# burn-research/OpenMEASURE

Measured on AMD Instinct MI355X. Metric: SPR fit+reconstruct throughput (GB/s snapshot matrix), higher is better.
Workload: dtype f64

## Files before the change

### include/spr_hip.h

```cpp
#ifndef SPR_HIP_H
#define SPR_HIP_H

#include <stddef.h>
#include <stdint.h>

#ifdef __cplusplus
extern "C" {
#endif

#define SPR_OK 0
#define SPR_E_INVALID (-1)
#define SPR_E_UNSUPPORTED (-2)
#define SPR_E_HIP (-3)
#define SPR_E_WORKSPACE (-4)

#define SPR_MAX_M 256
#define SPR_MAX_M_WIDE 512
#define SPR_MAX_R 128
#define SPR_MAX_R_STREAM 256
#define SPR_MAX_R_WIDE 1024

#define SPR_ABI_VERSION 5
int spr_abi_version(void);
const char *spr_last_error(void);
int spr_device_cus(int *out_cus);
int spr_upload_bytes(void *d_dst, const void *h_pinned_src, int64_t n_bytes, void *stream);
int spr_download_bytes(void *h_pinned_dst, const void *d_src, int64_t n_bytes, void *h_pinned_ticket, uint64_t ticket_value,
                       void *stream);
int spr_host_tridiag_vectors(const double *h_d, const double *h_e, int32_t m, const double *h_lam, int32_t r, double *h_Z,
                             int32_t iterations);
int spr_host_eig_top(const double *h_G, int32_t m, int32_t r, double *h_lam, double *h_V, void *fn_dsytrd, void *fn_dsterf,
                     void *fn_dormtr);
int spr_host_svd_top(const double *h_M, int32_t m, int32_t r, double *h_S, double *h_V, void *fn_dgebrd, void *fn_dbdsdc,
                     void *fn_dormbr);

size_t spr_stats_gram_workspace(int32_t m, int32_t n_features);
int spr_stats_gram_f64(const double *d_X, int64_t n_rows, int32_t m, int64_t ldx,
                       int64_t row0, int64_t n_points, int32_t n_features, int32_t center,
                       double *d_rowmean, void *d_workspace, size_t workspace_bytes, void *stream);
int spr_stats_gram_finalize_f64(int64_t n_rows, int32_t m, int64_t row0, int64_t n_points,
                                int32_t n_features, const void *d_workspace, size_t workspace_bytes,
                                double *d_fstats, double *d_gram, int32_t ldg, int32_t origin,
                                void *stream);
size_t spr_rowstats_workspace(int32_t n_features);
int spr_rowstats_f64(const double *d_X, int64_t n_rows, int32_t m, int64_t ldx, int64_t row0,
                     int64_t n_points, int32_t n_features, double *d_rowmean, double *d_fstats,
                     void *d_workspace, size_t workspace_bytes, void *stream);
size_t spr_gram_cross_workspace(int32_t m, int32_t n_features);
int spr_gram_cross_f64(const double *d_X, int64_t n_rows, int32_t m, int64_t ldx, int64_t row0,
                       int64_t n_points, int32_t n_features, int32_t center, double *d_rowmean,
                       double *d_gram, void *d_workspace, size_t workspace_bytes, void *stream);
int spr_rowmean_stats_f64(const double *d_rowmean, int64_t n_rows, int64_t row0, int64_t n_points,
                          int32_t n_features, double *d_fstats, void *d_workspace, size_t workspace_bytes,
                          void *stream);
int spr_gram_cross_pair_f64(const double *d_X, int64_t n_rows, int32_t col_a, int32_t col_b, int32_t w_b,
                            int32_t ldg, int64_t ldx, int64_t row0, int64_t n_points, int32_t n_features,
                            int32_t center, double *d_rowmean, double *d_gram, void *d_workspace,
                            size_t workspace_bytes, void *stream);

int32_t spr_spectrum_max_m(void);
int spr_spectrum_f64(const double *d_gram, const double *d_fstats_all, int32_t n_ranks,
                     int32_t n_features, int32_t m, int32_t scale_code, int32_t r, double *d_feat,
                     double *d_scale, double *d_inv_scale, double *d_lam, double *d_S, double *d_expvar,
                     double *d_V, double *d_W, double *d_Ar, double *d_info, void *stream);

int spr_gram_combine_f64(const double *d_gram, const double *d_fstats_all, int32_t n_ranks,
                         int32_t n_features, int32_t m, int32_t scale_code, double *d_G, double *d_feat,
                         double *d_scale, double *d_inv_scale, void *stream);

int spr_stats_gram_shifted_f64(const double *d_X, int64_t n_rows, int32_t m, int64_t ldx, int64_t row0,
                               int64_t n_points, int32_t n_features, const double *d_shift, double *d_rowsum,
                               void *d_workspace, size_t workspace_bytes, void *stream);
int spr_gram_shift_finish_f64(double *d_rowmean, const double *d_rowsum_b, int64_t n_rows, int32_t w_a, int32_t m,
                              double *d_gram, int32_t n_features, void *stream);

int spr_project_f64(const double *d_X, int64_t n_rows, int32_t m, int64_t ldx,
// ... 275 lines not shown
```

### openmeasure_amd/_lib.py

```python
from __future__ import annotations

import ctypes as C
import os

_HERE = os.path.dirname(os.path.abspath(__file__))
LIB_PATH = os.environ.get('SPR_HIP_LIBRARY') or os.path.join(_HERE, 'libspr_hip.so')

SPR_ABI_VERSION = 5
SPR_MAX_M = 256
SPR_MAX_M_WIDE = 512
SPR_MAX_R = 128
SPR_MAX_R_STREAM = 256
SPR_MAX_R_WIDE = 1024

_i32, _i64, _u64, _sz = C.c_int32, C.c_int64, C.c_uint64, C.c_size_t
_p = C.c_void_p
_dbl = C.c_double

PROTOTYPES = {
    'spr_abi_version': (C.c_int, []),
    'spr_last_error': (C.c_char_p, []),
    'spr_device_cus': (C.c_int, [C.POINTER(C.c_int)]),
    'spr_upload_bytes': (C.c_int, [_p, _p, _i64, _p]),
    'spr_download_bytes': (C.c_int, [_p, _p, _i64, _p, _u64, _p]),
    'spr_host_tridiag_vectors': (C.c_int, [_p, _p, _i32, _p, _i32, _p, _i32]),
    'spr_host_eig_top': (C.c_int, [_p, _i32, _i32, _p, _p, _p, _p, _p]),
    'spr_host_svd_top': (C.c_int, [_p, _i32, _i32, _p, _p, _p, _p, _p]),
    'spr_stats_gram_workspace': (_sz, [_i32, _i32]),
    'spr_stats_gram_f64': (C.c_int, [_p, _i64, _i32, _i64, _i64, _i64, _i32, _i32, _p, _p, _sz, _p]),
    'spr_stats_gram_finalize_f64': (C.c_int, [_i64, _i32, _i64, _i64, _i32, _p, _sz, _p, _p, _i32, _i32, _p]),
    'spr_stats_gram_shifted_f64': (C.c_int, [_p, _i64, _i32, _i64, _i64, _i64, _i32, _p, _p, _p, _sz, _p]),
    'spr_gram_shift_finish_f64': (C.c_int, [_p, _p, _i64, _i32, _i32, _p, _i32, _p]),
    'spr_rowstats_workspace': (_sz, [_i32]),
    'spr_rowstats_f64': (C.c_int, [_p, _i64, _i32, _i64, _i64, _i64, _i32, _p, _p, _p, _sz, _p]),
    'spr_gram_cross_workspace': (_sz, [_i32, _i32]),
    'spr_gram_cross_f64': (C.c_int, [_p, _i64, _i32, _i64, _i64, _i64, _i32, _i32, _p, _p, _p, _sz, _p]),
    'spr_gram_cross_pair_f64': (C.c_int, [_p, _i64, _i32, _i32, _i32, _i32, _i64, _i64, _i64, _i32, _i32, _p, _p, _p, _sz, _p]),
    'spr_rowmean_stats_f64': (C.c_int, [_p, _i64, _i64, _i64, _i32, _p, _p, _sz, _p]),
    'spr_spectrum_max_m': (_i32, []),
    'spr_spectrum_f64': (C.c_int, [_p, _p, _i32, _i32, _i32, _i32, _i32, _p, _p, _p, _p, _p, _p, _p, _p, _p, _p, _p]),
    'spr_gram_combine_f64': (C.c_int, [_p, _p, _i32, _i32, _i32, _i32, _p, _p, _p, _p, _p]),
    'spr_project_f64': (C.c_int, [_p, _i64, _i32, _i64, _i64, _i64, _i32, _i32, _p, _p, _p, _i32, _p, _i64, _i32, _p]),
    'spr_project_norms_supported': (_i32, [_i32, _i32, _i64, _i64, _p, _i32]),
    'spr_project_norms_f64': (C.c_int, [_p, _i64, _i32, _i64, _i64, _i64, _i32, _i32, _p, _p, _p, _i32, _p, _i64, _p, _p]),
    'spr_project_stream_norms_f64': (C.c_int, [_p, _i64, _i32, _i64, _i64, _i64, _i32, _i32, _p, _p, _p, _i32, _p, _i64, _p, _p, _sz, _p]),
    'spr_project_stream_workspace': (_sz, [_i32, _i32, _i32]),
    'spr_project_stream_f64': (C.c_int, [_p, _i64, _i32, _i64, _i64, _i64, _i32, _i32, _p, _p, _p, _i32, _p, _i64, _p, _sz, _p]),
    'spr_scale_rows_f64': (C.c_int, [_p, _i64, _i32, _i64, _i64, _i64, _i32, _p, _p, _p, _i64, _p]),
    'spr_unscale_f64': (C.c_int, [_p, _i64, _i64, _i64, _i32, _p, _p, _p, _p, _p]),
    'spr_feature_minmax_workspace': (_sz, [_i32]),
    'spr_feature_minmax_f64': (C.c_int, [_p, _i64, _i32, _i64, _i64, _i64, _i32, _p, _p, _sz, _p]),
    'spr_feature_digit_hist_f64': (C.c_int, [_p, _i64, _i32, _i64, _i64, _i64, _i32, _p, _i32, _i32, _i32, _p, _p]),
    'spr_colsums_workspace': (_sz, [_i32, _i32]),
    'spr_colsums_f64': (C.c_int, [_p, _i64, _i32, _i64, _i64, _i64, _i32, _p, _p, _p, _sz, _p]),
    'spr_fill_feature_f64': (C.c_int, [_p, _i64, _i64, _i64, _i32, _p, _p]),
    'spr_reconstruct_f64': (C.c_int, [_p, _i64, _i32, _i64, _i64, _i64, _i32, _p, _p, _p, _p, _i32, _p, _i64, _p]),
    'spr_bound_sweep_workspace': (_sz, [_i32, _i32]),
    'spr_bound_sweep_f64': (C.c_int, [_p, _i64, _i32, _i64, _i64, _i64, _i32, _p, _p, _p, _p, _p, _i32, _dbl, _i32, _p, _p, _sz, _p]),
    'spr_field_unstage_f64': (C.c_int, [_p, _i32, _i32, _i64, _p, _i64, _p]),
    'spr_field_unstage_blocks_f64': (C.c_int, [_p, _i32, _i32, _i64, _p, _p, _i64, _p]),
    'spr_p2p_handle_bytes': (_sz, []),
    'spr_p2p_alloc': (C.c_int, [_sz, _i32, _p, _p]),
    'spr_p2p_free': (C.c_int, [_p]),
# ... 109 lines not shown
```

### openmeasure_amd/csrc/common.hpp

```cpp
#pragma once
#include <hip/hip_runtime.h>
#include <stdint.h>
#include <stdio.h>

#include "spr_hip.h"

typedef double f64x4 __attribute__((ext_vector_type(4)));
typedef double f64x2 __attribute__((ext_vector_type(2)));

void spr_set_error(const char *fmt, ...);

#define SPR_REQUIRE(cond, code, ...)      \
  do {                                    \
    if (!(cond)) {                        \
      spr_set_error(__VA_ARGS__);         \
      return (code);                      \
    }                                     \
  } while (0)

#define SPR_HIP_TRY(expr)                                                          \
  do {                                                                             \
    hipError_t e__ = (expr);                                                       \
    if (e__ != hipSuccess) {                                                       \
      spr_set_error("%s failed: %s (%s:%d)", #expr, hipGetErrorString(e__),       \
// ... 42 lines not shown
__host__ __device__ inline int seg_first_feature(const SegPlan &p) { return (int)(p.row0 / p.n_points); }
__host__ __device__ inline int seg_last_feature(const SegPlan &p) {
  int64_t f = (p.row0 + p.n_rows - 1) / p.n_points;
  if (f > p.n_features - 1) f = p.n_features - 1;
  return (int)f;
}

inline int seg_total_wgs(const SegPlan &p) {
  int tot = 0;
  for (int f = seg_first_feature(p); f <= seg_last_feature(p); ++f) {
    int64_t lo, hi;
    seg_range(p, f, lo, hi);
    tot += seg_wgs(p, hi - lo);
  }
  return tot;
}

__device__ inline bool seg_locate(const SegPlan &p, int b, int &f, int &wl, int &wpf, int &base,
                                  int64_t &lo, int64_t &hi) {
  int acc = 0;
  int f1 = seg_last_feature(p);
  for (int ff = seg_first_feature(p); ff <= f1; ++ff) {
    seg_range(p, ff, lo, hi);
    int w = seg_wgs(p, hi - lo);
    if (b < acc + w) {
      f = ff; wl = b - acc; wpf = w; base = acc;
      return true;
    }
    acc += w;
  }
  return false;
}

template <int CTRL>
__device__ inline double dpp_f64(double v) {
  union { double d; int i[2]; } a, b;
  a.d = v;
  b.i[0] = __builtin_amdgcn_update_dpp(0, a.i[0], CTRL, 0xF, 0xF, true);
  b.i[1] = __builtin_amdgcn_update_dpp(0, a.i[1], CTRL, 0xF, 0xF, true);
  return b.d;
}

template <int WIDTH>
__device__ inline double group_sum_t(double v) {
  if (WIDTH >= 2) v += dpp_f64<0xB1>(v);
  if (WIDTH >= 4) v += dpp_f64<0x4E>(v);
  if (WIDTH >= 8) v += dpp_f64<0x141>(v);
  if (WIDTH >= 16) v += dpp_f64<0x140>(v);
  if (WIDTH >= 32) v += __shfl_xor(v, 16, 64);
  if (WIDTH >= 64) v += __shfl_xor(v, 32, 64);
  return v;
}

__device__ inline double group_sum(double v, int width) {
  for (int o = width >> 1; o > 0; o >>= 1) v += __shfl_xor(v, o, 64);
  return v;
}

constexpr int spr_pow2_divisor_le64(int n) {
  int p = 1;
  while (p < 64 && n % (2 * p) == 0) p *= 2;
  return p;
}

inline int spr_round_mt(int m) {
  static const int sup[] = {1, 2, 3, 4, 6, 8, 12, 16};
// ... 6 lines not shown
```

### openmeasure_amd/csrc/runtime.hip

```cpp
#include <stdarg.h>
#include <stdlib.h>
#include <string.h>

#include "common.hpp"

namespace {
thread_local char g_err[512] = "";
}

void spr_set_error(const char *fmt, ...) {
  va_list ap;
  va_start(ap, fmt);
  vsnprintf(g_err, sizeof(g_err), fmt, ap);
  va_end(ap);
}

int spr_cached_cus() {
  static int cus = 0;
  if (cus) return cus;
  int dev = 0;
  hipDeviceProp_t prop;
  if (hipGetDevice(&dev) != hipSuccess || hipGetDeviceProperties(&prop, dev) != hipSuccess) return 0;
  cus = prop.multiProcessorCount;
  if (const char *e = getenv("SPR_RESERVE_CUS")) {
    const int k = atoi(e);
    if (k > 0 && k < cus) cus -= k;
  }
  return cus;
}

extern "C" int spr_abi_version(void) { return SPR_ABI_VERSION; }

extern "C" const char *spr_last_error(void) { return g_err; }

extern "C" int spr_device_cus(int *out_cus) {
  SPR_REQUIRE(out_cus != nullptr, SPR_E_INVALID, "spr_device_cus: NULL output");
  const int c = spr_cached_cus();
  SPR_REQUIRE(c > 0, SPR_E_HIP, "spr_device_cus: no HIP device");
  *out_cus = c;
  return SPR_OK;
}

namespace {
__global__ __launch_bounds__(256) void upload_kernel(const uint64_t *__restrict__ src, uint64_t *__restrict__ dst,
                                                     int64_t n_words) {
  for (int64_t i = (int64_t)blockIdx.x * 256 + threadIdx.x; i < n_words; i += (int64_t)gridDim.x * 256)
    dst[i] = __builtin_nontemporal_load(src + i);
}
}

extern "C" int spr_upload_bytes(void *d_dst, const void *h_pinned_src, int64_t n_bytes, void *stream) {
  SPR_REQUIRE(d_dst && h_pinned_src, SPR_E_INVALID, "spr_upload_bytes: NULL pointer");
  SPR_REQUIRE(n_bytes > 0 && n_bytes % 8 == 0, SPR_E_INVALID, "spr_upload_bytes: n_bytes=%lld must be a positive multiple of 8",
              (long long)n_bytes);
  SPR_REQUIRE(((uintptr_t)d_dst | (uintptr_t)h_pinned_src) % 8 == 0, SPR_E_INVALID, "spr_upload_bytes: unaligned pointer");
  const int64_t words = n_bytes / 8;
  int64_t blocks = (words + 255) / 256;
  if (blocks > 64) blocks = 64;
  hipLaunchKernelGGL(upload_kernel, dim3((unsigned)blocks), dim3(256), 0, static_cast<hipStream_t>(stream),
                     static_cast<const uint64_t *>(h_pinned_src), static_cast<uint64_t *>(d_dst), words);
  SPR_LAUNCH_CHECK();
  return SPR_OK;
}

namespace {
__global__ __launch_bounds__(1024) void download_kernel(const uint64_t *__restrict__ src, uint64_t *__restrict__ dst,
                                                        int64_t n_words, unsigned long long *__restrict__ ticket,
                                                        unsigned long long value) {
  for (int64_t i = threadIdx.x; i < n_words; i += 1024) __builtin_nontemporal_store(src[i], dst + i);
  __builtin_amdgcn_fence(__ATOMIC_RELEASE, "");
  __syncthreads();
  if (threadIdx.x == 0) __hip_atomic_store(ticket, value, __ATOMIC_RELEASE, __HIP_MEMORY_SCOPE_SYSTEM);
}
// ... 16 lines not shown
```

### openmeasure_amd/csrc/stats_gram.hip

```cpp
#include <stdlib.h>

#include <type_traits>

#include "rowtile.hpp"

#ifndef GRAM_UNIT_PAIRING
#define GRAM_UNIT_PAIRING 1
#endif
#ifndef GRAM_ABLATE
#define GRAM_ABLATE 0
#endif
#if GRAM_ABLATE == 1
#define GRAM_MFMA(a, b, c) ({ asm volatile("" ::"v"(a), "v"(b)); (c); })
#else
#define GRAM_MFMA(a, b, c) __builtin_amdgcn_mfma_f64_16x16x4f64((a), (b), (c), 0, 0, 0)
#endif

namespace {

template <int MT>
struct GramShape {
  static constexpr int MPAD = 16 * MT;
  static constexpr int MP = MPAD + ((MT % 2 == 0) ? 16 : 0);
  static constexpr int T = MT * (MT + 1) / 2;
  static constexpr int NU = (MT + 1) / 2;
};

template <int MT> struct GramCfg;
template <> struct GramCfg<1>  { static constexpr int NW = 8,  R = 64, KS = 8; static constexpr bool DBUF = true; static constexpr int LPRMAX = 16; };
template <> struct GramCfg<2>  { static constexpr int NW = 8,  R = 32, KS = 8; static constexpr bool DBUF = true; static constexpr int LPRMAX = 16; };
template <> struct GramCfg<3>  { static constexpr int NW = 8,  R = 64, KS = 4; static constexpr bool DBUF = true; static constexpr int LPRMAX = 16; };
#ifndef GRAM4_R
#define GRAM4_R 64
#define GRAM4_LPR 8
#endif
template <> struct GramCfg<4>  { static constexpr int NW = 8,  R = GRAM4_R, KS = 4; static constexpr bool DBUF = true; static constexpr int LPRMAX = GRAM4_LPR; };
template <> struct GramCfg<6>  { static constexpr int NW = 12, R = 48, KS = 4; static constexpr bool DBUF = true; static constexpr int LPRMAX = 16; };
template <> struct GramCfg<8>  { static constexpr int NW = 8,  R = 32, KS = 2; static constexpr bool DBUF = true; static constexpr int LPRMAX = 16; };
template <> struct GramCfg<12> { static constexpr int NW = 12, R = 24, KS = 2; static constexpr bool DBUF = false; static constexpr int LPRMAX = 32; };
#ifndef GRAM_DBUF16
#define GRAM_DBUF16 false
#endif
template <> struct GramCfg<16> { static constexpr int NW = 8,  R = 32, KS = 1; static constexpr bool DBUF = GRAM_DBUF16; static constexpr int LPRMAX = 16; };

template <int MT> struct GramOut { static constexpr int KSO = (GramCfg<MT>::KS >= 4) ? 1 : GramCfg<MT>::KS; };

constexpr int tri_index(int mt, int ti, int tj) { return ti * mt - ti * (ti - 1) / 2 + (tj - ti); }

template <int MT>
__device__ inline void tile_coords(int idx, int &ti, int &tj) {
  ti = 0;
  while (ti < MT - 1 && idx >= MT - ti) { idx -= MT - ti; ++ti; }
  tj = ti + idx;
  if (tj > MT - 1) tj = MT - 1;
}

template <int MT, int U, int VEC, typename TX>
__device__ inline void gram_wave(const TX *__restrict__ X, int64_t ldx, int m, int center,
                                 int64_t lo, int64_t hi, int wl, int wpf, int ks, int wave, int lane,
                                 double *__restrict__ lds0, double *__restrict__ lds1,
                                 double *__restrict__ rowmean, double *__restrict__ stat_part,
                                 double *__restrict__ slab, double *__restrict__ rowsum) {
  using S = GramShape<MT>;
  using C = GramCfg<MT>;
  constexpr int R = C::R, KS = C::KS, NW = C::NW, MP = S::MP, T = S::T;
  constexpr int KROWS = R / KS, KSTEPS = KROWS / 4;
  constexpr int RA = U, RB = MT - 1 - U;
  constexpr int NA = MT - RA;
  constexpr int NB = (RB != RA) ? MT - RB : 0;
  static_assert(KROWS % 4 == 0, "k slice must be a multiple of the MFMA depth");
  using RT = RowTile<MT, R, MP, NW, C::LPRMAX, TX>;

  f64x4 accA[NA];
  f64x4 accB[NB > 0 ? NB : 1];
#pragma unroll
  for (int j = 0; j < NA; ++j) accA[j] = (f64x4){0.0, 0.0, 0.0, 0.0};
#pragma unroll
  for (int j = 0; j < NB; ++j) accB[j] = (f64x4){0.0, 0.0, 0.0, 0.0};

  RowStats st;
  st.init();
  RT tile;

  const int64_t nchunks = (hi - lo + R - 1) / R;
  int64_t c = wl;
  const double *mean_in = rowmean;
  tile.template load<VEC>(X, ldx, m, lo + c * R, hi, wave, lane, mean_in);
  tile.template center_store<true>(lds0, m, center, lo + c * R, hi, wave, lane, rowmean, &st, rowsum);
  int64_t cn = c + wpf;
  int64_t nrow0 = (cn < nchunks) ? lo + cn * R : hi;
  tile.template load<VEC>(X, ldx, m, nrow0, hi, wave, lane, mean_in);
  int buf = 0;
  const int frag = (lane >> 4) * MP + (lane & 15) + ks * KROWS * MP + RA * 16;
  while (c < nchunks) {
    double *cur = buf ? lds1 : lds0;
// ... 57 lines not shown
  if constexpr (KSO != KS) {
    static_assert((size_t)T * 256 <= (size_t)2 * R * MP, "tile staging must fit the panel buffers");
    double *red = lds0 + lane;
    for (int s = KS - 1; s >= 1; --s) {
      __syncthreads();
      if (ks == s) {
#pragma unroll
        for (int j = 0; j < NA; ++j) {
          double *tp = red + tri_index(MT, RA, RA + j) * 256;
          tp[0] = accA[j].x; tp[64] = accA[j].y; tp[128] = accA[j].z; tp[192] = accA[j].w;
        }
#pragma unroll
        for (int j = 0; j < NB; ++j) {
          double *tp = red + tri_index(MT, RB, RB + j) * 256;
          tp[0] = accB[j].x; tp[64] = accB[j].y; tp[128] = accB[j].z; tp[192] = accB[j].w;
        }
      }
      __syncthreads();
      if (ks == s - 1) {
#pragma unroll
        for (int j = 0; j < NA; ++j) {
          const double *tp = red + tri_index(MT, RA, RA + j) * 256;
          accA[j].x += tp[0]; accA[j].y += tp[64]; accA[j].z += tp[128]; accA[j].w += tp[192];
        }
#pragma unroll
        for (int j = 0; j < NB; ++j) {
          const double *tp = red + tri_index(MT, RB, RB + j) * 256;
          accB[j].x += tp[0]; accB[j].y += tp[64]; accB[j].z += tp[128]; accB[j].w += tp[192];
        }
      }
    }
  }
  if (KSO == KS || ks == 0) {
    double *sp = slab + ((int64_t)blockIdx.x * KSO + (KSO == KS ? ks : 0)) * T * 256 + lane;
#pragma unroll
    for (int j = 0; j < NA; ++j) {
      double *tp = sp + (int64_t)tri_index(MT, RA, RA + j) * 256;
      tp[0] = accA[j].x; tp[64] = accA[j].y; tp[128] = accA[j].z; tp[192] = accA[j].w;
    }
#pragma unroll
    for (int j = 0; j < NB; ++j) {
      double *tp = sp + (int64_t)tri_index(MT, RB, RB + j) * 256;
      tp[0] = accB[j].x; tp[64] = accB[j].y; tp[128] = accB[j].z; tp[192] = accB[j].w;
    }
  }
  if ((lane % RT::LPR) == 0) {
    double *q = stat_part + ((int64_t)blockIdx.x * RT::ROWS_PER_IT + wave * RT::RPW + lane / RT::LPR) * 3;
    q[0] = st.cnt; q[1] = st.mean(); q[2] = st.m2();
  }
}

__device__ inline void chan_merge(double &n, double &mu, double &m2, double nb, double mb, double sb) {
  if (nb > 0.0) {
    const double tot = n + nb, d = mb - mu;
    mu += d * nb / tot;
    m2 += sb + d * d * n * nb / tot;
    n = tot;
  }
}

template <int MT, int U, typename TX, bool EXT, bool SUMS>
__device__ inline void gram_wave_own(const TX *__restrict__ X, int64_t ldx, int64_t lo, int64_t hi, int wl, int wpf, int ks,
                                     int wave, int lane, double *__restrict__ lds0, double *__restrict__ lds1,
                                     double *__restrict__ rowmean, double *__restrict__ slab, double *__restrict__ rowsum) {
  using S = GramShape<MT>;
  using C = GramCfg<MT>;
  constexpr int R = C::R, KS = C::KS, NW = C::NW, MP = S::MP, T = S::T;
  constexpr int KROWS = R / KS, KSTEPS = KROWS / 4;
  constexpr int RA = U, RB = MT - 1 - U;
  constexpr int NA = MT - RA;
  constexpr int NB = (RB != RA) ? MT - RB : 0;
  using RT = RowTile<MT, R, MP, NW, C::LPRMAX, TX>;

  f64x4 accA[NA];
  f64x4 accB[NB > 0 ? NB : 1];
#pragma unroll
  for (int j = 0; j < NA; ++j) accA[j] = (f64x4){0.0, 0.0, 0.0, 0.0};
#pragma unroll
  for (int j = 0; j < NB; ++j) accB[j] = (f64x4){0.0, 0.0, 0.0, 0.0};

  RT tile;
  const int64_t nchunks = (hi - lo + R - 1) / R;
  const int64_t lane_off = (int64_t)(wave * RT::RPW + lane / RT::LPR) * ldx;
  auto base_of = [&](int64_t row0) { return X + row0 * ldx; };
  int64_t c = wl;
  int64_t crow0 = lo + c * R;
#pragma unroll
  for (int it = 0; it < RT::IT; ++it) tile.template load_pass_own<EXT>(it, base_of(crow0), ldx, lane_off, hi - crow0, wave, lane, rowmean, crow0);
  if (crow0 + R <= hi) {
#pragma unroll
    for (int it = 0; it < RT::IT; ++it) tile.template center_store_own<true, EXT, SUMS>(it, lds0, crow0, hi - crow0, wave, lane, rowmean, rowsum);
  } else {
#pragma unroll
    for (int it = 0; it < RT::IT; ++it) tile.template center_store_own<false, EXT, SUMS>(it, lds0, crow0, hi - crow0, wave, lane, rowmean, rowsum);
  }
  int64_t cn = c + wpf;
  int64_t nrow0 = (cn < nchunks) ? lo + cn * R : hi;
// ... 23 lines not shown
      double op[2][NA];
#pragma unroll
      for (int j = 0; j < NA; ++j) op[0][j] = p[16 * j];
#pragma unroll
      for (int k = 0; k < KSTEPS; ++k) {
        if (k + 1 < KSTEPS) {
#pragma unroll
          for (int j = 0; j < NA; ++j) op[(k + 1) & 1][j] = p[(k + 1) * 4 * MP + 16 * j];
        }
#pragma unroll
        for (int j = 0; j < NA; ++j) accA[j] = GRAM_MFMA(op[k & 1][0], op[k & 1][j], accA[j]);
#pragma unroll
        for (int j = 0; j < NB; ++j) accB[j] = GRAM_MFMA(op[k & 1][RB - RA], op[k & 1][RB - RA + j], accB[j]);
        if (nfull) stage(std::true_type{}, k); else stage(std::false_type{}, k);
      }
    } else {
#pragma unroll
      for (int k = 0; k < KSTEPS; ++k) {
        double op[NA];
#pragma unroll
        for (int j = 0; j < NA; ++j) op[j] = p[k * 4 * MP + 16 * j];
#pragma unroll
        for (int j = 0; j < NA; ++j) accA[j] = GRAM_MFMA(op[0], op[j], accA[j]);
#pragma unroll
        for (int j = 0; j < NB; ++j) accB[j] = GRAM_MFMA(op[RB - RA], op[RB - RA + j], accB[j]);
        if (nfull) stage(std::true_type{}, k); else stage(std::false_type{}, k);
      }
    }
    buf ^= 1;
    c = cn;
    cn = c2;
    nrow0 = n2row0;
  }
  double *sp = slab + ((int64_t)blockIdx.x * KS + ks) * T * 256 + lane;
#pragma unroll
  for (int j = 0; j < NA; ++j) {
    double *tp = sp + (int64_t)tri_index(MT, RA, RA + j) * 256;
    tp[0] = accA[j].x; tp[64] = accA[j].y; tp[128] = accA[j].z; tp[192] = accA[j].w;
  }
#pragma unroll
  for (int j = 0; j < NB; ++j) {
    double *tp = sp + (int64_t)tri_index(MT, RB, RB + j) * 256;
    tp[0] = accB[j].x; tp[64] = accB[j].y; tp[128] = accB[j].z; tp[192] = accB[j].w;
  }
}

template <int MT, typename TX, bool EXT, bool SUMS>
__global__ __launch_bounds__(GramCfg<MT>::NW * 64) void stats_gram_own_kernel(
    const TX *__restrict__ X, int64_t ldx, SegPlan plan, double *__restrict__ rowmean, double *__restrict__ slab,
    double *__restrict__ rowsum) {
  using S = GramShape<MT>;
  using C = GramCfg<MT>;
  constexpr int NU = S::NU;
  __shared__ double lds[2][C::R * S::MP];
  int f, wl, wpf, base;
  int64_t lo, hi;
  if (!seg_locate(plan, blockIdx.x, f, wl, wpf, base, lo, hi)) return;
  const int lane = threadIdx.x & 63;
  const int wave = __builtin_amdgcn_readfirstlane(threadIdx.x >> 6);
  const int ks = wave / NU;
  const int unit = (GRAM_UNIT_PAIRING && NU == 8 && C::KS == 1) ? ((wave < 4) ? wave : 11 - wave) : wave % NU;
#define GRAM_UNIT(UV)                                                                                          \
  case UV:                                                                                                     \
    if constexpr (UV < NU)                                                                                     \
      gram_wave_own<MT, UV, TX, EXT, SUMS>(X, ldx, lo, hi, wl, wpf, ks, wave, lane, lds[0], lds[1], rowmean, slab, rowsum); \
    break;
  switch (unit) {
    GRAM_UNIT(0) GRAM_UNIT(1) GRAM_UNIT(2) GRAM_UNIT(3) GRAM_UNIT(4) GRAM_UNIT(5) GRAM_UNIT(6) GRAM_UNIT(7)
    default: break;
  }
#undef GRAM_UNIT
}

constexpr int RS_THREADS = 1024;
__global__ __launch_bounds__(RS_THREADS) void gram_rowmean_stats_kernel(const double *__restrict__ rowmean, SegPlan plan,
                                                                        int slots_per_wg, double *__restrict__ stat_part) {
  __shared__ double sn[RS_THREADS / 64], smu[RS_THREADS / 64], sm2[RS_THREADS / 64];
  int f, wl, wpf, base;
  int64_t lo, hi;
  if (!seg_locate(plan, blockIdx.x, f, wl, wpf, base, lo, hi)) return;
  const int lane = threadIdx.x & 63, wave = threadIdx.x >> 6;
  RowStats st;
  st.init();
  const int64_t step = (int64_t)wpf * RS_THREADS;
  int64_t row = lo + (int64_t)wl * RS_THREADS + threadIdx.x;
  for (; row + 3 * step < hi; row += 4 * step) {
    const double a = rowmean[row], b = rowmean[row + step], c = rowmean[row + 2 * step], d = rowmean[row + 3 * step];
    st.push(a, true); st.push(b, true); st.push(c, true); st.push(d, true);
  }
  for (; row < hi; row += step) st.push(rowmean[row], true);
  double n = st.cnt, mu = st.mean(), m2 = st.m2();
  for (int o = 32; o > 0; o >>= 1) {
    const double on = __shfl_down(n, o, 64), om = __shfl_down(mu, o, 64), os = __shfl_down(m2, o, 64);
    chan_merge(n, mu, m2, on, om, os);
  }
  if (lane == 0) { sn[wave] = n; smu[wave] = mu; sm2[wave] = m2; }
  __syncthreads();
  double *q = stat_part + (int64_t)blockIdx.x * slots_per_wg * 3;
  if (threadIdx.x == 0) {
    n = 0.0; mu = 0.0; m2 = 0.0;
    for (int w = 0; w < RS_THREADS / 64; ++w) chan_merge(n, mu, m2, sn[w], smu[w], sm2[w]);
    q[0] = n; q[1] = mu; q[2] = m2;
  }
  for (int e = 3 + threadIdx.x; e < slots_per_wg * 3; e += RS_THREADS) q[e] = 0.0;
}

template <int MT, int VEC, typename TX>
__global__ __launch_bounds__(GramCfg<MT>::NW * 64) void stats_gram_kernel(
    const TX *__restrict__ X, int64_t ldx, int m, int center_i, SegPlan plan,
    double *__restrict__ rowmean, double *__restrict__ stat_part, double *__restrict__ slab, double *__restrict__ rowsum) {
  using S = GramShape<MT>;
  using C = GramCfg<MT>;
  constexpr int NU = S::NU;
  static_assert(NU * C::KS == C::NW, "waves = units x k slices");
  __shared__ double lds[2][C::R * S::MP];

  int f, wl, wpf, base;
  int64_t lo, hi;
  if (!seg_locate(plan, blockIdx.x, f, wl, wpf, base, lo, hi)) return;

  const int lane = threadIdx.x & 63;
  const int wave = __builtin_amdgcn_readfirstlane(threadIdx.x >> 6);
  const int unit = wave % NU, ks = wave / NU;
#define GRAM_UNIT(UV)                                                                                        \
  case UV:                                                                                                   \
    if constexpr (UV < NU)                                                                                   \
      gram_wave<MT, UV, VEC, TX>(X, ldx, m, center_i, lo, hi, wl, wpf, ks, wave, lane, lds[0],    \
                        lds[1], rowmean, stat_part, slab, rowsum);                                           \
    break;
  switch (unit) {
    GRAM_UNIT(0) GRAM_UNIT(1) GRAM_UNIT(2) GRAM_UNIT(3) GRAM_UNIT(4) GRAM_UNIT(5) GRAM_UNIT(6) GRAM_UNIT(7)
    default: break;
  }
#undef GRAM_UNIT
}

template <int MT>
__global__ __launch_bounds__(1024) void gram_finalize_kernel(
    const double *__restrict__ slab, const double *__restrict__ stat_part, int m, SegPlan plan,
    int slots_per_wg, double *__restrict__ gram, double *__restrict__ fstats, int ldg, int origin) {
  constexpr int T = GramShape<MT>::T;
  constexpr int KS = GramOut<MT>::KSO;
  __shared__ double red[4][256];
  const int f = blockIdx.y;
  const int tile = blockIdx.x;
  int base = 0, wpf = 0;
  {
    int acc = 0;
    const int f0 = seg_first_feature(plan), f1 = seg_last_feature(plan);
    for (int ff = f0; ff <= f1; ++ff) {
      int64_t lo, hi;
      seg_range(plan, ff, lo, hi);
      const int w = seg_wgs(plan, hi - lo);
      if (ff == f) { base = acc; wpf = w; }
      acc += w;
    }
  }
  int ti, tj;
  tile_coords<MT>(tile, ti, tj);
  const int e = threadIdx.x & 255, g = threadIdx.x >> 8;
  const int np = wpf * KS;
  const double *sp = slab + ((int64_t)base * KS * T + tile) * 256 + e;
  const int64_t stride = (int64_t)T * 256;
  double s0 = 0.0, s1 = 0.0, s2 = 0.0, s3 = 0.0;
  int p = g;
  for (; p + 12 < np; p += 16) {
    s0 += sp[p * stride];
    s1 += sp[(p + 4) * stride];
    s2 += sp[(p + 8) * stride];
    s3 += sp[(p + 12) * stride];
  }
  for (; p < np; p += 4) s0 += sp[p * stride];
  red[g][e] = (s0 + s1) + (s2 + s3);
  __syncthreads();
  if (g == 0) {
    const double sum = (red[0][e] + red[1][e]) + (red[2][e] + red[3][e]);
    const int l = e & 63, reg = e >> 6;
    const int gi = ti * 16 + (l >> 4) + 4 * reg, gj = tj * 16 + (l & 15);
    if (gi < m && gj < m) {
      double *G = gram + (int64_t)f * ldg * ldg + (int64_t)origin * ldg + origin;
      G[(int64_t)gi * ldg + gj] = sum;
      if (ti != tj) G[(int64_t)gj * ldg + gi] = sum;
    }
  }
  if (tile == 0) {
    __syncthreads();
    double n = 0.0, mu = 0.0, m2 = 0.0;
    const double *q = stat_part + (int64_t)base * slots_per_wg * 3;
    const int tot_slots = wpf * slots_per_wg;
    for (int pp = threadIdx.x; pp < tot_slots; pp += 1024) chan_merge(n, mu, m2, q[3 * pp], q[3 * pp + 1], q[3 * pp + 2]);
    double *sn = &red[0][0], *smu = &red[1][0], *sm2 = &red[2][0];
    for (int o = 32; o > 0; o >>= 1) {
      const double on = __shfl_down(n, o, 64), om = __shfl_down(mu, o, 64), os = __shfl_down(m2, o, 64);
      chan_merge(n, mu, m2, on, om, os);
    }
    const int w = threadIdx.x >> 6;
    if ((threadIdx.x & 63) == 0) { sn[w] = n; smu[w] = mu; sm2[w] = m2; }
    __syncthreads();
    if (threadIdx.x == 0) {
      n = 0.0; mu = 0.0; m2 = 0.0;
      for (int ww = 0; ww < 16; ++ww) chan_merge(n, mu, m2, sn[ww], smu[ww], sm2[ww]);
      fstats[3 * f] = n; fstats[3 * f + 1] = mu; fstats[3 * f + 2] = m2;
    }
  }
}

template <int MT>
int occupancy_wgs() {
  static int cached = 0;
  if (cached) return cached;
  int per_cu = 0;
  if (hipOccupancyMaxActiveBlocksPerMultiprocessor(&per_cu, stats_gram_kernel<MT, 2, double>, GramCfg<MT>::NW * 64, 0) != hipSuccess ||
      per_cu < 1)
    per_cu = 1;
  if (per_cu > 4) per_cu = 4;
  const int cus = spr_cached_cus();
  cached = per_cu * (cus > 0 ? cus : 256);
  return cached;
}

template <int MT>
SegPlan make_plan(int64_t n_rows, int64_t row0, int64_t n_points, int32_t n_features) {
  SegPlan p;
  p.row0 = row0; p.n_rows = n_rows; p.n_points = n_points; p.n_features = n_features;
  p.total_wg = occupancy_wgs<MT>();
  p.chunk_rows = GramCfg<MT>::R;
  return p;
}

template <int MT>
size_t workspace_bytes(int32_t n_features) {
  using RT = RowTile<MT, GramCfg<MT>::R, GramShape<MT>::MP, GramCfg<MT>::NW, GramCfg<MT>::LPRMAX>;
  const int64_t max_grid = (int64_t)occupancy_wgs<MT>() + n_features;
  return (size_t)max_grid * GramCfg<MT>::KS * GramShape<MT>::T * 256 * sizeof(double) +
         (size_t)max_grid * RT::ROWS_PER_IT * 3 * sizeof(double);
}

template <int MT, typename TX>
int launch(const TX *X, int64_t n_rows, int32_t m, int64_t ldx, int64_t row0, int64_t n_points,
           int32_t n_features, int center, double *rowmean, void *ws, size_t ws_bytes, hipStream_t st,
           double *rowsum = nullptr) {
  SPR_REQUIRE(ws_bytes >= workspace_bytes<MT>(n_features), SPR_E_WORKSPACE,
              "spr_stats_gram_f64: workspace %zu < %zu", ws_bytes, workspace_bytes<MT>(n_features));
  SPR_REQUIRE(!rowsum || center == 2, SPR_E_INVALID, "spr_stats_gram: row sums are an output of centre mode 2 only");
  SegPlan plan = make_plan<MT>(n_rows, row0, n_points, n_features);
  const int grid = seg_total_wgs(plan);
  const int64_t max_grid = (int64_t)occupancy_wgs<MT>() + n_features;
  SPR_REQUIRE(grid >= 1 && grid <= max_grid, SPR_E_INVALID, "spr_stats_gram_f64: bad grid %d", grid);
  double *slab = static_cast<double *>(ws);
  double *stat_part = slab + (size_t)max_grid * GramCfg<MT>::KS * GramShape<MT>::T * 256;
  const int vec_ok = (m % 2 == 0) && (ldx % 2 == 0) && ((reinterpret_cast<uintptr_t>(X) & (2 * sizeof(TX) - 1)) == 0);
  const int lm = vec_ok ? ((m == 16 * MT) ? 2 : 1) : 0;
#define SG_LAUNCH(LM)                                                                                         \
  hipLaunchKernelGGL((stats_gram_kernel<MT, LM, TX>), dim3(grid), dim3(GramCfg<MT>::NW * 64), 0, st, X, ldx, (int)m, \
                     center, plan, rowmean, stat_part, slab, rowsum)
  using RTL = RowTile<MT, GramCfg<MT>::R, GramShape<MT>::MP, GramCfg<MT>::NW, GramCfg<MT>::LPRMAX, TX>;
  static const bool own_on = [] { const char *e = getenv("SPR_GRAM_OWN"); return !(e && e[0] == '0'); }();
  if (MT >= 8 && lm == 2 && (center == 1 || center == 2) && own_on && (sizeof(TX) * ldx) % 16 == 0 &&
      (reinterpret_cast<uintptr_t>(X) & 15) == 0) {
    if constexpr (MT >= 8) {
      if (center == 1)
        hipLaunchKernelGGL((stats_gram_own_kernel<MT, TX, false, false>), dim3(grid), dim3(GramCfg<MT>::NW * 64), 0, st, X, ldx,
                           plan, rowmean, slab, rowsum);
      else if (!rowsum)
        hipLaunchKernelGGL((stats_gram_own_kernel<MT, TX, true, false>), dim3(grid), dim3(GramCfg<MT>::NW * 64), 0, st, X, ldx,
                           plan, rowmean, slab, rowsum);
      else
        hipLaunchKernelGGL((stats_gram_own_kernel<MT, TX, true, true>), dim3(grid), dim3(GramCfg<MT>::NW * 64), 0, st, X, ldx,
                           plan, rowmean, slab, rowsum);
      SPR_LAUNCH_CHECK();
      hipLaunchKernelGGL(gram_rowmean_stats_kernel, dim3(grid), dim3(RS_THREADS), 0, st, rowmean, plan, (int)RTL::ROWS_PER_IT,
                         stat_part);
      SPR_LAUNCH_CHECK();
      return SPR_OK;
    }
  }
  if (lm == 2) SG_LAUNCH(2);
  else if (lm == 1) SG_LAUNCH(1);
  else SG_LAUNCH(0);
// ... 137 lines not shown
```

Baseline: 1173.

## Balance Gram row split across workgroups independent of feature boundaries

Replaces the per-feature segmented work assignment with an even panel-based row split across workgroups, where each workgroup walks the feature pieces its range crosses and writes partials to per-part slots. Finalize and rowmean-stats kernels gather partials via the new slot mapping. This aims to remove load imbalance when features have uneven workgroup counts, at the cost of extra syncthreads between parts and indirect slot indexing in reductions. Only applies to balanced configurations (MT>=8 with full k-slice output).

```diff
diff --git a/include/spr_hip.h b/include/spr_hip.h
--- a/include/spr_hip.h
+++ b/include/spr_hip.h
@@ -42,6 +42,11 @@
                                 int32_t n_features, const void *d_workspace, size_t workspace_bytes,
                                 double *d_fstats, double *d_gram, int32_t ldg, int32_t origin,
                                 void *stream);
+int spr_row_split_parts(int64_t row0, int64_t n_rows, int64_t n_points, int32_t n_features, int32_t total_wg,
+                        int32_t panel_rows, int32_t b, int32_t capacity, int64_t *h_lo, int64_t *h_hi, int32_t *h_feature,
+                        int32_t *h_slot);
+int spr_row_split_feature_slots(int64_t row0, int64_t n_rows, int64_t n_points, int32_t n_features, int32_t total_wg,
+                                int32_t panel_rows, int32_t f, int32_t capacity, int32_t *h_slot);
 size_t spr_rowstats_workspace(int32_t n_features);
 int spr_rowstats_f64(const double *d_X, int64_t n_rows, int32_t m, int64_t ldx, int64_t row0,
                      int64_t n_points, int32_t n_features, double *d_rowmean, double *d_fstats,
diff --git a/openmeasure_amd/_lib.py b/openmeasure_amd/_lib.py
--- a/openmeasure_amd/_lib.py
+++ b/openmeasure_amd/_lib.py
@@ -29,6 +29,8 @@
     'spr_stats_gram_workspace': (_sz, [_i32, _i32]),
     'spr_stats_gram_f64': (C.c_int, [_p, _i64, _i32, _i64, _i64, _i64, _i32, _i32, _p, _p, _sz, _p]),
     'spr_stats_gram_finalize_f64': (C.c_int, [_i64, _i32, _i64, _i64, _i32, _p, _sz, _p, _p, _i32, _i32, _p]),
+    'spr_row_split_parts': (C.c_int, [_i64, _i64, _i64, _i32, _i32, _i32, _i32, _i32, _p, _p, _p, _p]),
+    'spr_row_split_feature_slots': (C.c_int, [_i64, _i64, _i64, _i32, _i32, _i32, _i32, _i32, _p]),
     'spr_stats_gram_shifted_f64': (C.c_int, [_p, _i64, _i32, _i64, _i64, _i64, _i32, _p, _p, _p, _sz, _p]),
     'spr_gram_shift_finish_f64': (C.c_int, [_p, _p, _i64, _i32, _i32, _p, _i32, _p]),
     'spr_rowstats_workspace': (_sz, [_i32]),
diff --git a/openmeasure_amd/csrc/common.hpp b/openmeasure_amd/csrc/common.hpp
--- a/openmeasure_amd/csrc/common.hpp
+++ b/openmeasure_amd/csrc/common.hpp
@@ -98,6 +98,67 @@
   return false;
 }
 
+__host__ __device__ inline int64_t split_panels(const SegPlan &p) { return (p.n_rows + p.chunk_rows - 1) / p.chunk_rows; }
+__host__ __device__ inline int split_wgs(const SegPlan &p) {
+  const int64_t np = split_panels(p);
+  return (int)(np < p.total_wg ? np : p.total_wg);
+}
+__host__ __device__ inline int64_t split_cut(const SegPlan &p, int w, int b) {
+  const int64_t row = ((int64_t)b * split_panels(p) / w) * p.chunk_rows;
+  return row < p.n_rows ? row : p.n_rows;
+}
+
+struct SplitPart {
+  int64_t lo, hi;
+  int32_t feature;
+  int32_t slot;
+};
+struct SplitIter {
+  int64_t pos, end;
+  int32_t b, w, f;
+};
+__host__ __device__ inline bool split_begin(const SegPlan &p, int b, SplitIter &it) {
+  it.w = split_wgs(p);
+  if (b < 0 || b >= it.w) return false;
+  it.b = b;
+  it.pos = split_cut(p, it.w, b);
+  it.end = split_cut(p, it.w, b + 1);
+  it.f = (int32_t)((p.row0 + it.pos) / p.n_points);
+  return it.pos < it.end;
+}
+__host__ __device__ inline bool split_next(const SegPlan &p, SplitIter &it, SplitPart &q) {
+  if (it.pos >= it.end) return false;
+  const int64_t fhi = (int64_t)(it.f + 1) * p.n_points - p.row0;
+  q.lo = it.pos;
+  q.hi = fhi < it.end ? fhi : it.end;
+  q.feature = it.f;
+  q.slot = (q.hi == it.end) ? it.b : it.w + (it.f - seg_first_feature(p));
+  it.pos = q.hi;
+  ++it.f;
+  return true;
+}
+
+__host__ __device__ inline int split_first_ending_after(const SegPlan &p, int w, int64_t row) {
+  int a = 0, z = w;
+  while (a < z) {
+    const int mid = (a + z) >> 1;
+    if (split_cut(p, w, mid + 1) > row) z = mid; else a = mid + 1;
+  }
+  return a;
+}
+__host__ __device__ inline void split_feature_slots(const SegPlan &p, int f, int &b0, int &nb, int &extra) {
+  int64_t lo, hi;
+  seg_range(p, f, lo, hi);
+  b0 = 0; nb = 0; extra = -1;
+  if (f < 0 || f >= p.n_features || hi <= lo) return;
+  const int w = split_wgs(p);
+  b0 = split_first_ending_after(p, w, lo);
+  const int b1 = split_first_ending_after(p, w, hi);
+  nb = b1 - b0;
+  if (b1 < w && split_cut(p, w, b1) < hi) extra = w + (f - seg_first_feature(p));
+}
+__host__ __device__ inline int split_slot_at(int b0, int nb, int extra, int i) { return i < nb ? b0 + i : extra; }
+
 template <int CTRL>
 __device__ inline double dpp_f64(double v) {
   union { double d; int i[2]; } a, b;
diff --git a/openmeasure_amd/csrc/runtime.hip b/openmeasure_amd/csrc/runtime.hip
--- a/openmeasure_amd/csrc/runtime.hip
+++ b/openmeasure_amd/csrc/runtime.hip
@@ -39,6 +39,50 @@
   SPR_REQUIRE(c > 0, SPR_E_HIP, "spr_device_cus: no HIP device");
   *out_cus = c;
   return SPR_OK;
+}
+
+extern "C" int spr_row_split_parts(int64_t row0, int64_t n_rows, int64_t n_points, int32_t n_features, int32_t total_wg,
+                                   int32_t panel_rows, int32_t b, int32_t capacity, int64_t *h_lo, int64_t *h_hi,
+                                   int32_t *h_feature, int32_t *h_slot) {
+  SPR_REQUIRE(n_rows > 0 && n_points > 0 && n_features > 0 && row0 >= 0 && total_wg > 0 && panel_rows > 0 && b >= 0 && capacity >= 0,
+              SPR_E_INVALID, "spr_row_split_parts: bad plan row0=%lld n_rows=%lld n_points=%lld n_features=%d total_wg=%d panel_rows=%d b=%d",
+              (long long)row0, (long long)n_rows, (long long)n_points, n_features, total_wg, panel_rows, b);
+  SPR_REQUIRE(n_rows <= n_points * (int64_t)n_features - row0, SPR_E_INVALID,
+              "spr_row_split_parts: rows [%lld,%lld) exceed n_points*n_features=%lld", (long long)row0,
+              (long long)(row0 + n_rows), (long long)(n_points * (int64_t)n_features));
+  SPR_REQUIRE(capacity == 0 || (h_lo && h_hi && h_feature && h_slot), SPR_E_INVALID, "spr_row_split_parts: NULL output");
+  SegPlan p;
+  p.row0 = row0; p.n_rows = n_rows; p.n_points = n_points; p.n_features = n_features;
+  p.total_wg = total_wg; p.chunk_rows = panel_rows;
+  SplitIter it;
+  if (!split_begin(p, b, it)) return 0;
+  SplitPart q;
+  int n = 0;
+  while (split_next(p, it, q)) {
+    if (n < capacity) { h_lo[n] = q.lo; h_hi[n] = q.hi; h_feature[n] = q.feature; h_slot[n] = q.slot; }
+    ++n;
+  }
+  return n;
+}
+
+extern "C" int spr_row_split_feature_slots(int64_t row0, int64_t n_rows, int64_t n_points, int32_t n_features, int32_t total_wg,
+                                           int32_t panel_rows, int32_t f, int32_t capacity, int32_t *h_slot) {
+  SPR_REQUIRE(n_rows > 0 && n_points > 0 && n_features > 0 && row0 >= 0 && total_wg > 0 && panel_rows > 0 && f >= 0 &&
+                  f < n_features && capacity >= 0,
+              SPR_E_INVALID, "spr_row_split_feature_slots: bad plan row0=%lld n_rows=%lld n_points=%lld n_features=%d total_wg=%d panel_rows=%d f=%d",
+              (long long)row0, (long long)n_rows, (long long)n_points, n_features, total_wg, panel_rows, f);
+  SPR_REQUIRE(n_rows <= n_points * (int64_t)n_features - row0, SPR_E_INVALID,
+              "spr_row_split_feature_slots: rows [%lld,%lld) exceed n_points*n_features=%lld", (long long)row0,
+              (long long)(row0 + n_rows), (long long)(n_points * (int64_t)n_features));
+  SPR_REQUIRE(capacity == 0 || h_slot, SPR_E_INVALID, "spr_row_split_feature_slots: NULL output");
+  SegPlan p;
+  p.row0 = row0; p.n_rows = n_rows; p.n_points = n_points; p.n_features = n_features;
+  p.total_wg = total_wg; p.chunk_rows = panel_rows;
+  int b0, nb, extra;
+  split_feature_slots(p, f, b0, nb, extra);
+  const int n = nb + (extra >= 0 ? 1 : 0);
+  for (int i = 0; i < n && i < capacity; ++i) h_slot[i] = split_slot_at(b0, nb, extra, i);
+  return n;
 }
 
 namespace {
diff --git a/openmeasure_amd/csrc/stats_gram.hip b/openmeasure_amd/csrc/stats_gram.hip
--- a/openmeasure_amd/csrc/stats_gram.hip
+++ b/openmeasure_amd/csrc/stats_gram.hip
@@ -45,6 +45,8 @@
 
 template <int MT> struct GramOut { static constexpr int KSO = (GramCfg<MT>::KS >= 4) ? 1 : GramCfg<MT>::KS; };
 
+template <int MT> struct GramBalanced { static constexpr bool value = (MT >= 8) && (GramOut<MT>::KSO == GramCfg<MT>::KS); };
+
 constexpr int tri_index(int mt, int ti, int tj) { return ti * mt - ti * (ti - 1) / 2 + (tj - ti); }
 
 template <int MT>
@@ -60,7 +62,7 @@
                                  int64_t lo, int64_t hi, int wl, int wpf, int ks, int wave, int lane,
                                  double *__restrict__ lds0, double *__restrict__ lds1,
                                  double *__restrict__ rowmean, double *__restrict__ stat_part,
-                                 double *__restrict__ slab, double *__restrict__ rowsum) {
+                                 double *__restrict__ slab, double *__restrict__ rowsum, int slot) {
   using S = GramShape<MT>;
   using C = GramCfg<MT>;
   constexpr int R = C::R, KS = C::KS, NW = C::NW, MP = S::MP, T = S::T;
@@ -184,7 +186,7 @@
     }
   }
   if (KSO == KS || ks == 0) {
-    double *sp = slab + ((int64_t)blockIdx.x * KSO + (KSO == KS ? ks : 0)) * T * 256 + lane;
+    double *sp = slab + ((int64_t)slot * KSO + (KSO == KS ? ks : 0)) * T * 256 + lane;
 #pragma unroll
     for (int j = 0; j < NA; ++j) {
       double *tp = sp + (int64_t)tri_index(MT, RA, RA + j) * 256;
@@ -197,7 +199,7 @@
     }
   }
   if ((lane % RT::LPR) == 0) {
-    double *q = stat_part + ((int64_t)blockIdx.x * RT::ROWS_PER_IT + wave * RT::RPW + lane / RT::LPR) * 3;
+    double *q = stat_part + ((int64_t)slot * RT::ROWS_PER_IT + wave * RT::RPW + lane / RT::LPR) * 3;
     q[0] = st.cnt; q[1] = st.mean(); q[2] = st.m2();
   }
 }
@@ -214,7 +216,8 @@
 template <int MT, int U, typename TX, bool EXT, bool SUMS>
 __device__ inline void gram_wave_own(const TX *__restrict__ X, int64_t ldx, int64_t lo, int64_t hi, int wl, int wpf, int ks,
                                      int wave, int lane, double *__restrict__ lds0, double *__restrict__ lds1,
-                                     double *__restrict__ rowmean, double *__restrict__ slab, double *__restrict__ rowsum) {
+                                     double *__restrict__ rowmean, double *__restrict__ slab, double *__restrict__ rowsum,
+                                     int slot) {
   using S = GramShape<MT>;
   using C = GramCfg<MT>;
   constexpr int R = C::R, KS = C::KS, NW = C::NW, MP = S::MP, T = S::T;
@@ -304,7 +307,7 @@
     cn = c2;
     nrow0 = n2row0;
   }
-  double *sp = slab + ((int64_t)blockIdx.x * KS + ks) * T * 256 + lane;
+  double *sp = slab + ((int64_t)slot * KS + ks) * T * 256 + lane;
 #pragma unroll
   for (int j = 0; j < NA; ++j) {
     double *tp = sp + (int64_t)tri_index(MT, RA, RA + j) * 256;
@@ -324,10 +327,10 @@
   using S = GramShape<MT>;
   using C = GramCfg<MT>;
   constexpr int NU = S::NU;
+  static_assert(GramBalanced<MT>::value, "the own-means lane walks the balanced split");
   __shared__ double lds[2][C::R * S::MP];
-  int f, wl, wpf, base;
-  int64_t lo, hi;
-  if (!seg_locate(plan, blockIdx.x, f, wl, wpf, base, lo, hi)) return;
+  SplitIter it;
+  if (!split_begin(plan, blockIdx.x, it)) return;
   const int lane = threadIdx.x & 63;
   const int wave = __builtin_amdgcn_readfirstlane(threadIdx.x >> 6);
   const int ks = wave / NU;
@@ -335,11 +338,17 @@
 #define GRAM_UNIT(UV)                                                                                          \
   case UV:                                                                                                     \
     if constexpr (UV < NU)                                                                                     \
-      gram_wave_own<MT, UV, TX, EXT, SUMS>(X, ldx, lo, hi, wl, wpf, ks, wave, lane, lds[0], lds[1], rowmean, slab, rowsum); \
+      gram_wave_own<MT, UV, TX, EXT, SUMS>(X, ldx, q.lo, q.hi, 0, 1, ks, wave, lane, lds[0], lds[1], rowmean, slab, rowsum, \
+                                           q.slot);                                                            \
     break;
-  switch (unit) {
-    GRAM_UNIT(0) GRAM_UNIT(1) GRAM_UNIT(2) GRAM_UNIT(3) GRAM_UNIT(4) GRAM_UNIT(5) GRAM_UNIT(6) GRAM_UNIT(7)
-    default: break;
+  SplitPart q;
+  for (bool more = split_next(plan, it, q); more;) {
+    switch (unit) {
+      GRAM_UNIT(0) GRAM_UNIT(1) GRAM_UNIT(2) GRAM_UNIT(3) GRAM_UNIT(4) GRAM_UNIT(5) GRAM_UNIT(6) GRAM_UNIT(7)
+      default: break;
+    }
+    more = split_next(plan, it, q);
+    if (more) __syncthreads();
   }
 #undef GRAM_UNIT
 }
@@ -348,33 +357,37 @@
 __global__ __launch_bounds__(RS_THREADS) void gram_rowmean_stats_kernel(const double *__restrict__ rowmean, SegPlan plan,
                                                                         int slots_per_wg, double *__restrict__ stat_part) {
   __shared__ double sn[RS_THREADS / 64], smu[RS_THREADS / 64], sm2[RS_THREADS / 64];
-  int f, wl, wpf, base;
-  int64_t lo, hi;
-  if (!seg_locate(plan, blockIdx.x, f, wl, wpf, base, lo, hi)) return;
+  SplitIter it;
+  if (!split_begin(plan, blockIdx.x, it)) return;
   const int lane = threadIdx.x & 63, wave = threadIdx.x >> 6;
-  RowStats st;
-  st.init();
-  const int64_t step = (int64_t)wpf * RS_THREADS;
-  int64_t row = lo + (int64_t)wl * RS_THREADS + threadIdx.x;
-  for (; row + 3 * step < hi; row += 4 * step) {
-    const double a = rowmean[row], b = rowmean[row + step], c = rowmean[row + 2 * step], d = rowmean[row + 3 * step];
-    st.push(a, true); st.push(b, true); st.push(c, true); st.push(d, true);
-  }
-  for (; row < hi; row += step) st.push(rowmean[row], true);
-  double n = st.cnt, mu = st.mean(), m2 = st.m2();
-  for (int o = 32; o > 0; o >>= 1) {
-    const double on = __shfl_down(n, o, 64), om = __shfl_down(mu, o, 64), os = __shfl_down(m2, o, 64);
-    chan_merge(n, mu, m2, on, om, os);
-  }
-  if (lane == 0) { sn[wave] = n; smu[wave] = mu; sm2[wave] = m2; }
-  __syncthreads();
-  double *q = stat_part + (int64_t)blockIdx.x * slots_per_wg * 3;
-  if (threadIdx.x == 0) {
-    n = 0.0; mu = 0.0; m2 = 0.0;
-    for (int w = 0; w < RS_THREADS / 64; ++w) chan_merge(n, mu, m2, sn[w], smu[w], sm2[w]);
-    q[0] = n; q[1] = mu; q[2] = m2;
-  }
-  for (int e = 3 + threadIdx.x; e < slots_per_wg * 3; e += RS_THREADS) q[e] = 0.0;
+  SplitPart part;
+  while (split_next(plan, it, part)) {
+    const int64_t hi = part.hi;
+    RowStats st;
+    st.init();
+    const int64_t step = RS_THREADS;
+    int64_t row = part.lo + threadIdx.x;
+    for (; row + 3 * step < hi; row += 4 * step) {
+      const double a = rowmean[row], b = rowmean[row + step], c = rowmean[row + 2 * step], d = rowmean[row + 3 * step];
+      st.push(a, true); st.push(b, true); st.push(c, true); st.push(d, true);
+    }
+    for (; row < hi; row += step) st.push(rowmean[row], true);
+    double n = st.cnt, mu = st.mean(), m2 = st.m2();
+    for (int o = 32; o > 0; o >>= 1) {
+      const double on = __shfl_down(n, o, 64), om = __shfl_down(mu, o, 64), os = __shfl_down(m2, o, 64);
+      chan_merge(n, mu, m2, on, om, os);
+    }
+    if (lane == 0) { sn[wave] = n; smu[wave] = mu; sm2[wave] = m2; }
+    __syncthreads();
+    double *q = stat_part + (int64_t)part.slot * slots_per_wg * 3;
+    if (threadIdx.x == 0) {
+      n = 0.0; mu = 0.0; m2 = 0.0;
+      for (int w = 0; w < RS_THREADS / 64; ++w) chan_merge(n, mu, m2, sn[w], smu[w], sm2[w]);
+      q[0] = n; q[1] = mu; q[2] = m2;
+    }
+    for (int e = 3 + threadIdx.x; e < slots_per_wg * 3; e += RS_THREADS) q[e] = 0.0;
+    __syncthreads();
+  }
 }
 
 template <int MT, int VEC, typename TX>
@@ -387,10 +400,6 @@
   static_assert(NU * C::KS == C::NW, "waves = units x k slices");
   __shared__ double lds[2][C::R * S::MP];
 
-  int f, wl, wpf, base;
-  int64_t lo, hi;
-  if (!seg_locate(plan, blockIdx.x, f, wl, wpf, base, lo, hi)) return;
-
   const int lane = threadIdx.x & 63;
   const int wave = __builtin_amdgcn_readfirstlane(threadIdx.x >> 6);
   const int unit = wave % NU, ks = wave / NU;
@@ -398,11 +407,31 @@
   case UV:                                                                                                   \
     if constexpr (UV < NU)                                                                                   \
       gram_wave<MT, UV, VEC, TX>(X, ldx, m, center_i, lo, hi, wl, wpf, ks, wave, lane, lds[0],    \
-                        lds[1], rowmean, stat_part, slab, rowsum);                                           \
+                        lds[1], rowmean, stat_part, slab, rowsum, slot);                                     \
     break;
-  switch (unit) {
-    GRAM_UNIT(0) GRAM_UNIT(1) GRAM_UNIT(2) GRAM_UNIT(3) GRAM_UNIT(4) GRAM_UNIT(5) GRAM_UNIT(6) GRAM_UNIT(7)
-    default: break;
+  if constexpr (GramBalanced<MT>::value) {
+    SplitIter it;
+    if (!split_begin(plan, blockIdx.x, it)) return;
+    SplitPart q;
+    for (bool more = split_next(plan, it, q); more;) {
+      const int64_t lo = q.lo, hi = q.hi;
+      const int wl = 0, wpf = 1, slot = q.slot;
+      switch (unit) {
+        GRAM_UNIT(0) GRAM_UNIT(1) GRAM_UNIT(2) GRAM_UNIT(3) GRAM_UNIT(4) GRAM_UNIT(5) GRAM_UNIT(6) GRAM_UNIT(7)
+        default: break;
+      }
+      more = split_next(plan, it, q);
+      if (more) __syncthreads();
+    }
+  } else {
+    int f, wl, wpf, base;
+    int64_t lo, hi;
+    if (!seg_locate(plan, blockIdx.x, f, wl, wpf, base, lo, hi)) return;
+    const int slot = blockIdx.x;
+    switch (unit) {
+      GRAM_UNIT(0) GRAM_UNIT(1) GRAM_UNIT(2) GRAM_UNIT(3) GRAM_UNIT(4) GRAM_UNIT(5) GRAM_UNIT(6) GRAM_UNIT(7)
+      default: break;
+    }
   }
 #undef GRAM_UNIT
 }
@@ -416,8 +445,10 @@
   __shared__ double red[4][256];
   const int f = blockIdx.y;
   const int tile = blockIdx.x;
-  int base = 0, wpf = 0;
-  {
+  int base = 0, wpf = 0, extra = -1;
+  if constexpr (GramBalanced<MT>::value) {
+    split_feature_slots(plan, f, base, wpf, extra);
+  } else {
     int acc = 0;
     const int f0 = seg_first_feature(plan), f1 = seg_last_feature(plan);
     for (int ff = f0; ff <= f1; ++ff) {
@@ -428,21 +459,23 @@
       acc += w;
     }
   }
+  const int nslots = wpf + (extra >= 0 ? 1 : 0);
   int ti, tj;
   tile_coords<MT>(tile, ti, tj);
   const int e = threadIdx.x & 255, g = threadIdx.x >> 8;
-  const int np = wpf * KS;
-  const double *sp = slab + ((int64_t)base * KS * T + tile) * 256 + e;
+  const int np = nslots * KS;
+  const double *sp0 = slab + (int64_t)tile * 256 + e;
   const int64_t stride = (int64_t)T * 256;
+  auto at = [&](int p) { return sp0[((int64_t)split_slot_at(base, wpf, extra, p / KS) * KS + p % KS) * stride]; };
   double s0 = 0.0, s1 = 0.0, s2 = 0.0, s3 = 0.0;
   int p = g;
   for (; p + 12 < np; p += 16) {
-    s0 += sp[p * stride];
-    s1 += sp[(p + 4) * stride];
-    s2 += sp[(p + 8) * stride];
-    s3 += sp[(p + 12) * stride];
-  }
-  for (; p < np; p += 4) s0 += sp[p * stride];
+    s0 += at(p);
+    s1 += at(p + 4);
+    s2 += at(p + 8);
+    s3 += at(p + 12);
+  }
+  for (; p < np; p += 4) s0 += at(p);
   red[g][e] = (s0 + s1) + (s2 + s3);
   __syncthreads();
   if (g == 0) {
@@ -458,9 +491,12 @@
   if (tile == 0) {
     __syncthreads();
     double n = 0.0, mu = 0.0, m2 = 0.0;
-    const double *q = stat_part + (int64_t)base * slots_per_wg * 3;
-    const int tot_slots = wpf * slots_per_wg;
-    for (int pp = threadIdx.x; pp < tot_slots; pp += 1024) chan_merge(n, mu, m2, q[3 * pp], q[3 * pp + 1], q[3 * pp + 2]);
+    const int tot_slots = nslots * slots_per_wg;
+    for (int pp = threadIdx.x; pp < tot_slots; pp += 1024) {
+      const double *q = stat_part +
+                        ((int64_t)split_slot_at(base, wpf, extra, pp / slots_per_wg) * slots_per_wg + pp % slots_per_wg) * 3;
+      chan_merge(n, mu, m2, q[0], q[1], q[2]);
+    }
     double *sn = &red[0][0], *smu = &red[1][0], *sm2 = &red[2][0];
     for (int o = 32; o > 0; o >>= 1) {
       const double on = __shfl_down(n, o, 64), om = __shfl_down(mu, o, 64), os = __shfl_down(m2, o, 64);
@@ -516,7 +552,7 @@
               "spr_stats_gram_f64: workspace %zu < %zu", ws_bytes, workspace_bytes<MT>(n_features));
   SPR_REQUIRE(!rowsum || center == 2, SPR_E_INVALID, "spr_stats_gram: row sums are an output of centre mode 2 only");
   SegPlan plan = make_plan<MT>(n_rows, row0, n_points, n_features);
-  const int grid = seg_total_wgs(plan);
+  const int grid = GramBalanced<MT>::value ? split_wgs(plan) : seg_total_wgs(plan);
   const int64_t max_grid = (int64_t)occupancy_wgs<MT>() + n_features;
   SPR_REQUIRE(grid >= 1 && grid <= max_grid, SPR_E_INVALID, "spr_stats_gram_f64: bad grid %d", grid);
   double *slab = static_cast<double *>(ws);
```

New measurement: 1179 (median of 6 runs). About the same (+0.5%).
